# abhilash1910/bitsandbytes-SYCL

Measured on AMD Instinct MI355X. Metric: NF4 matmul TFLOPS + INT8 igemmlt TOPS @ 4096x4096x11008, 1/2/4/8 GPU, higher is better.
Workload: dtype bf16; 1 GPU; NF4 Linear4bit GEMM M=4096 N=4096 K=11008 (functional.gemm_4bit on its static route for 4096 x 4096 x 11008: k_hgemm<bf16> (hand-written, hgemm.hip) after k_dequantize_4bit_stream<bf16,NF4>, every step dequantising its weight); M=4096, N=4096, K=11008, blocksize=64, quant_type=nf4, compress_statistics=True, parallelism=single GPU

## Files before the change

bitsandbytes-sycl_amd/csrc/common.hpp:

```cpp
#pragma once

#include <hip/hip_runtime.h>
#include <atomic>
#include <stdint.h>
#include <stdio.h>

typedef uint16_t bf16_t;
typedef _Float16 fp16_t;

namespace bnb {

template <typename T> using Knob = std::atomic<T>;

enum DataType { GENERAL8BIT = 0, FP4 = 1, NF4 = 2 };

hipStream_t current_stream();
void set_error(int code, const char* what);
#define BNB_LAUNCH_CHECK(name)                                              \
  do {                                                                      \
    hipError_t e_ = hipGetLastError();                                      \
    if (e_ != hipSuccess) ::bnb::set_error((int)e_, name);                  \
  } while (0)

template <typename T> struct Io;
template <> struct Io<float> {
  __device__ static __forceinline__ float to_f32(float v) { return v; }
  __device__ static __forceinline__ float from_f32(float v) { return v; }
};
__device__ __forceinline__ float opaque(float v) {
  asm volatile("" : "+v"(v));
  return v;
// ... 225 lines not shown
```

bitsandbytes-sycl_amd/csrc/hgemm.hip:

```cpp
#include "gemm_common.hpp"
#include "int8_common.hpp"

#include <algorithm>
#include <type_traits>
#include <utility>

namespace bnb {

constexpr int HG_BM = 256, HG_BN = 256, HG_THREADS = 256;

typedef float hg_f32x2_t __attribute__((ext_vector_type(2)));
typedef __bf16 hg_bf16x2_t __attribute__((ext_vector_type(2)));
typedef _Float16 hg_f16x2_t __attribute__((ext_vector_type(2)));
template <typename T> __device__ __forceinline__ uint32_t cvt_pk(float lo, float hi);
template <> __device__ __forceinline__ uint32_t cvt_pk<bf16_t>(float lo, float hi) {
  return __builtin_bit_cast(uint32_t, __builtin_convertvector((hg_f32x2_t){lo, hi}, hg_bf16x2_t));
}
template <> __device__ __forceinline__ uint32_t cvt_pk<fp16_t>(float lo, float hi) {
  return __builtin_bit_cast(uint32_t, __builtin_convertvector((hg_f32x2_t){lo, hi}, hg_f16x2_t));
}

enum HgOp { HG_BF16 = 0, HG_FP16 = 1, HG_I8_DEQ = 2 };
typedef unsigned hg_u32x4_t __attribute__((ext_vector_type(4)));
typedef int hg_i32x4_t __attribute__((ext_vector_type(4)));
// ... 35 lines not shown
    acc_t c;
    asm volatile("v_mfma_i32_16x16x64_i8 %0, %1, %2, 0" : "=a"(c) : "v"(a), "v"(b));
    return c;
  }
};

__device__ __forceinline__ void glds16_sv_m0(const void* sbase, uint32_t voff, uint32_t lds) {
  asm volatile("s_mov_b32 m0, %2\n\ts_nop 0\n\tglobal_load_lds_dwordx4 %0, %1" : : "v"(voff), "s"(sbase), "s"(lds) : "memory");
}

template <int STEP>
__device__ __forceinline__ void glds16_chain(const void* sbase, uint32_t voff) {
  asm volatile("global_load_lds_dwordx4 %0, %1\n\ts_add_u32 m0, m0, %2" : : "v"(voff), "s"(sbase), "i"(STEP) : "memory");
}
__device__ __forceinline__ void hg_set_m0(uint32_t lds) { asm volatile("s_mov_b32 m0, %0" : : "s"(lds) : "memory"); }

__device__ __forceinline__ int hg_swz(int r, int s) { return r * 128 + ((s ^ ((r >> 1) & 7)) << 4); }

__device__ __forceinline__ void glds4_sv_m0(const void* sbase, uint32_t voff, uint32_t lds) {
  asm volatile("s_mov_b32 m0, %2\n\ts_nop 0\n\tglobal_load_lds_dword %0, %1" : : "v"(voff), "s"(sbase), "s"(lds) : "memory");
}

__device__ __forceinline__ uint32_t mm_dequant_pair(int32_t a0, int32_t a1, float rs, float cs0, float cs1, float b0,
                                                    float b1) {
  hg_f32x2_t v = {(float)a0, (float)a1};
  v = v * (hg_f32x2_t){6.200012e-05f, 6.200012e-05f};
  v = v * (hg_f32x2_t){rs, rs};
  v = v * (hg_f32x2_t){cs0, cs1};
  asm volatile("" : "+v"(v));
  v = v + (hg_f32x2_t){b0, b1};
// ... 4 lines not shown
constexpr int HG_V = 16 + 8192;
constexpr int HG_V_CWT = 32768;
static Knob<int> g_hg_cwt{1};
constexpr int HG_V_EPI = 65536;
static Knob<int> g_hg_epi{1};
constexpr int HG_V_CNT = 131072;
constexpr int HG_V_TL = 262144;
__device__ unsigned long long* g_hg_tl = nullptr;
__device__ int g_hg_tl_nswap = 0;
__device__ int g_hg_tl_nostore = 0;
[[maybe_unused]] static int g_hg_tl_on = 0;
__device__ __forceinline__ unsigned long long hg_now() {
  unsigned long long t;
  asm volatile("s_memrealtime %0\n\ts_waitcnt lgkmcnt(0)" : "=s"(t)::"memory");
  return t;
}

template <class F, int... Q>
__device__ __forceinline__ void hg_static_for_impl(F&& f, std::integer_sequence<int, Q...>) {
  (f(std::integral_constant<int, Q>{}), ...);
}
template <int N, class F>
__device__ __forceinline__ void hg_static_for(F&& f) {
  hg_static_for_impl(f, std::make_integer_sequence<int, N>{});
}

template <int WI, int WJ> struct HgPlan3;
template <> struct HgPlan3<8, 8> {
  static constexpr int B1 = 21, B2 = 50, B3 = 88, SETB = 22, SETA = 61, VM = 13, SIDEQ = 120;
  __host__ __device__ static constexpr int wread(int q) { return q < 16 && (q & 1) == 0 ? q >> 1 : -1; }
// ... 235 lines not shown
  const int first_m = (wg / group_span) * GROUP;
  const int gsize = min(tilesM - first_m, GROUP);
  const int tm = first_m + (wg % group_span) % gsize;
  int tn = (wg % group_span) / gsize;
  if constexpr (TL) {
    if (g_hg_tl_nswap) tn = (tn + tilesN / 2) % tilesN;
  }
  const int m0 = tm * BM, n0 = tn * BN;

  uint32_t aoff[WI], boff[WJ];
  const uint32_t lda2 = (uint32_t)lda * E, ldb2 = (uint32_t)ldb * E;
#pragma unroll
  for (int i = 0; i < WI; ++i) {
    const int row = 8 * (WI * wave + i) + (lane >> 3);
    const uint32_t slot = (uint32_t)((lane & 7) ^ ((row >> 1) & 7));
    aoff[i] = (uint32_t)min(m0 + row, M - 1) * lda2 + 16u * slot;
  }
#pragma unroll
  for (int i = 0; i < WJ; ++i) {
    const int row = 8 * (WJ * wave + i) + (lane >> 3);
    const uint32_t slot = (uint32_t)((lane & 7) ^ ((row >> 1) & 7));
    boff[i] = (uint32_t)min(n0 + row, N - 1) * ldb2 + 16u * slot;
  }
  const uint32_t lds_base = __builtin_amdgcn_readfirstlane((uint32_t)(uintptr_t)smem);
  const uint32_t ldsA0 = lds_base + wave * WI * 1024, ldsB0 = lds_base + TA + wave * WJ * 1024;
  auto dma_a = [&](int kt, int st, int i) { glds16_sv_m0(A + (long long)kt * 128, aoff[i], ldsA0 + st * STG + i * 1024); };
  auto dma_b = [&](int kt, int st, int i) { glds16_sv_m0(B + (long long)kt * 128, boff[i], ldsB0 + st * STG + i * 1024); };

  const int wm = wave >> 1, wn = wave & 1;
  const int fr = lane & 15, fg = lane >> 4, key = (fr >> 1) & 7;
  const int xo0 = (16 * WI * wm + fr) * 128 + ((fg ^ key) << 4);
  const int xo1 = (16 * WI * wm + fr) * 128 + (((4 + fg) ^ key) << 4);
  const int wo0 = TA + (16 * WJ * wn + fr) * 128 + ((fg ^ key) << 4);
  const int wo1 = TA + (16 * WJ * wn + fr) * 128 + (((4 + fg) ^ key) << 4);
  using frag_t = hg_u32x4_t;
  auto rd = [&](int st, int off, int f) -> frag_t {
    return *reinterpret_cast<const frag_t*>(smem + st * STG + off + f * 2048);
// ... 82 lines not shown
        glds4_sv_m0(bias, 4u * (uint32_t)min(n0 / 2 + 64 * c + lane, N / 2 - 1), sb + 4 * BM + 4 * BN + 256 * c);
  }
#pragma unroll
  for (int i = 0; i < WI; ++i) dma_a(0, 0, i);
#pragma unroll
  for (int i = 0; i < WJ; ++i) dma_b(0, 0, i);
  const int k1 = min(1, nk - 1);
#pragma unroll
  for (int i = 0; i < WI; ++i) dma_a(k1, 1, i);
#pragma unroll
  for (int i = 0; i < WJ; ++i) dma_b(k1, 1, i);
  asm volatile("s_waitcnt vmcnt(%0)" ::"i"(WI + WJ) : "memory");
  if constexpr (SIDE) __builtin_amdgcn_s_waitcnt(0xC07F);
  __builtin_amdgcn_s_barrier();
  if constexpr (TL) tl1 = hg_now();
#pragma unroll
  for (int f = 0; f < WJ; ++f) w0[f] = rd(0, wo0, f);
#pragma unroll
  for (int f = 0; f < WI; ++f) x0[f] = rd(0, xo0, f);

  if (nk == 1) {
    tile3(std::true_type{}, std::true_type{}, 0);
  } else {
    tile3(std::true_type{}, std::false_type{}, 0);
    for (int t = 1; t + 1 < nk; ++t) tile3(std::false_type{}, std::false_type{}, t);
    tile3(std::false_type{}, std::true_type{}, nk - 1);
  }
  wait_vmcnt0();
  if constexpr (TL) tl2 = hg_now();
  __builtin_amdgcn_sched_barrier(0);
  asm volatile("s_nop 7\n\ts_nop 7\n\ts_nop 7" ::: "memory");
  __builtin_amdgcn_sched_barrier(0);
  if constexpr (SIDE) {
    auto consume = [&](int it) {
      side_words(it);
      side_stat();
#pragma unroll
      for (int j = 0; j < 4; ++j) {
// ... 61 lines not shown
#pragma unroll
      for (int i = 0; i < WI; ++i) rsv[i] = *reinterpret_cast<const float*>(sst + 4 * (rl + 16 * i));
#pragma unroll
      for (int j = 0; j < WJ; ++j) {
        csv[j] = *reinterpret_cast<const f32x4_t*>(sst + 4 * BM + 4 * (cl + 16 * j));
        if ((N & 1) == 0)
          bsv[j] = bias ? *reinterpret_cast<const uint2*>(sst + 4 * BM + 4 * BN + 2 * (cl + 16 * j)) : make_uint2(0u, 0u);
        else
          bsv[j] = bias ? *reinterpret_cast<const uint2*>(bias + nb + 16 * j) : make_uint2(0u, 0u);
      }
    }
    auto convert = [&](int i, int j) {
      uint2 v;
      if constexpr (OP == HG_BF16 || OP == HG_FP16) {
        using T = typename std::conditional<OP == HG_BF16, bf16_t, fp16_t>::type;
        v.x = cvt_pk<T>(acc[j][i][0], acc[j][i][1]);
        v.y = cvt_pk<T>(acc[j][i][2], acc[j][i][3]);
      } else if constexpr (OP == HG_I8_DEQ) {
        auto bf = [&](uint32_t w, int hi) { return (float)__builtin_bit_cast(fp16_t, (uint16_t)(w >> (16 * hi))); };
        v.x = mm_dequant_pair(acc[j][i][0], acc[j][i][1], rsv[i], csv[j][0], csv[j][1], bf(bsv[j].x, 0), bf(bsv[j].x, 1));
        v.y = mm_dequant_pair(acc[j][i][2], acc[j][i][3], rsv[i], csv[j][2], csv[j][3], bf(bsv[j].y, 0), bf(bsv[j].y, 1));
      }
      *reinterpret_cast<uint2*>(ep + (16 * i + (lane_e & 15)) * EPI_PITCH + 2 * (16 * j + 4 * (lane_e >> 4))) = v;
    };
    uint8_t* cbase = reinterpret_cast<uint8_t*>(Cv) + ((long long)(m0 + 16 * WI * wm) * ldc + n0 + 16 * WJ * wn) * 2;
    constexpr int CPR = 2 * WJ, RPI = 64 / CPR;
    auto store_rows = [&](int it) {
      const int row = RPI * it + lane_e / CPR, c16 = lane_e % CPR;
      const uint4 v = *reinterpret_cast<const uint4*>(ep + row * EPI_PITCH + 16 * c16);
      uint8_t* dst = cbase + (long long)row * ldc * 2 + 16 * c16;
      if constexpr ((V & HG_V_CWT) != 0)
        asm volatile("global_store_dwordx4 %0, %1, off sc1" : : "v"(dst), "v"((hg_u32x4_t){v.x, v.y, v.z, v.w}) : "memory");
      else
        *reinterpret_cast<uint4*>(dst) = v;
    };
    if ((V & HG_V_EPI) != 0 && (long long)ldc * 2 * 16 * WI < 0x7FFFFFFFLL) {
// ... 42 lines not shown
          __builtin_amdgcn_sched_barrier(0);
        }
      }
      __builtin_amdgcn_s_waitcnt(0xC07F);
#pragma unroll 8
      for (int it = 0; it < 16 * WI / RPI; ++it) store_rows(it);
    }
  } else if (!full) {
#pragma unroll
    for (int i = 0; i < WI; ++i) {
      const int m = mb + 16 * i;
      const long long mc = min(m, M - 1);
      float rs = 0.f;
      if constexpr (OP == HG_I8_DEQ) rs = rowStats[mc];
#pragma unroll
      for (int j = 0; j < WJ; ++j)
#pragma unroll
        for (int r = 0; r < 4; ++r) {
          const int n = nb + 16 * j + r;
          if (m < M && n < N) {
            if constexpr (OP == HG_BF16) reinterpret_cast<bf16_t*>(Cv)[mc * ldc + n] = Io<bf16_t>::from_f32(acc[j][i][r]);
            else if constexpr (OP == HG_FP16) reinterpret_cast<fp16_t*>(Cv)[mc * ldc + n] = Io<fp16_t>::from_f32(acc[j][i][r]);
            else
              reinterpret_cast<fp16_t*>(Cv)[mc * ldc + n] =
                  mm_dequant_value(acc[j][i][r], rs, colStats[n], bias ? (float)bias[n] : 0.0f);
          }
          __builtin_amdgcn_sched_barrier(0);
        }
    }
  }
  if constexpr ((V & HG_V_TAIL) != 0) {
    __builtin_amdgcn_s_barrier();
    hg_side_tail<T16>(side, smem + wave * (16 * WI * EPI_PITCH), lane_e, blockIdx.x * 4u + (uint32_t)wave,
                      gridDim.x * 4u);
  }
  if constexpr (TL) {
    const unsigned long long tl3 = hg_now();
    asm volatile("s_waitcnt vmcnt(0)" ::: "memory");
    const unsigned long long tl4 = hg_now();
    if (lane == 0 && g_hg_tl != nullptr) {
      unsigned long long* o = g_hg_tl + ((long long)blockIdx.x * 4 + wave) * 8;
      o[0] = tl0; o[1] = tl1; o[2] = tl2; o[3] = tl3; o[4] = tl4; o[5] = (unsigned long long)wgs;
      o[6] = (unsigned long long)(__builtin_amdgcn_s_getreg((3 << 11) | 20) & 15);
// ... 289 lines not shown
```

bitsandbytes-sycl_amd/csrc/quant.hip:

```cpp
#include "common.hpp"

#include <type_traits>

namespace bnb {


template <typename T> struct Load8;
template <> struct Load8<float> {
  __device__ static __forceinline__ void load(const float* p, float (&v)[8]) {
    const float4 a = *reinterpret_cast<const float4*>(p);
    const float4 b = *reinterpret_cast<const float4*>(p + 4);
    v[0] = a.x; v[1] = a.y; v[2] = a.z; v[3] = a.w; v[4] = b.x; v[5] = b.y; v[6] = b.z; v[7] = b.w;
  }
};
template <> struct Load8<fp16_t> {
  __device__ static __forceinline__ void load(const fp16_t* p, float (&v)[8]) {
    const uint4 u = *reinterpret_cast<const uint4*>(p);
    const uint32_t w[4] = {u.x, u.y, u.z, u.w};
#pragma unroll
    for (int i = 0; i < 4; ++i) {
      v[2 * i] = (float)__builtin_bit_cast(fp16_t, (uint16_t)(w[i] & 0xFFFF));
      v[2 * i + 1] = (float)__builtin_bit_cast(fp16_t, (uint16_t)(w[i] >> 16));
    }
  }
// ... 412 lines not shown
}

template <typename T, int DT>
bool dequantize_4bit_nested(const uint8_t* A, const uint8_t* q8, const float* code2, const float* absmax2,
                            const float* offset, T* out, int blocksize, int blocksize2, long long n) {
  if (n <= 0) return true;
  if (blocksize < 64 || (blocksize & (blocksize - 1)) || blocksize2 <= 0 || (blocksize2 & (blocksize2 - 1)) ||
      n % 8 != 0 || ((uintptr_t)A & 3) != 0 || !aligned16(out))
    return false;
  const NestedStats ns{q8, code2, absmax2, offset, __builtin_ctz(blocksize2)};
  launch_dq_stream<T, DT, true>(A, nullptr, out, __builtin_ctz(blocksize), n / 8, ns);
  BNB_LAUNCH_CHECK("dequantize_4bit_nested");
  return true;
}

__global__ void __launch_bounds__(256)
k_dequantize_nested_absmax(const float* __restrict__ code2, const uint8_t* __restrict__ q, const float* __restrict__ absmax2,
                           const float* __restrict__ offset, float* __restrict__ out, int bs2_shift, long long n) {
  __shared__ float c2[256];
  c2[threadIdx.x] = code2[threadIdx.x];
  const float off = *offset;
  __syncthreads();
  const long long i0 = 16 * ((long long)blockIdx.x * 256 + threadIdx.x);
  if (i0 >= n) return;
  if (i0 + 16 <= n && (((uintptr_t)(q + i0)) & 15) == 0 && (((uintptr_t)(out + i0)) & 15) == 0) {
    const uint4 v = *reinterpret_cast<const uint4*>(q + i0);
    const uint32_t w[4] = {v.x, v.y, v.z, v.w};
#pragma unroll
    for (int d = 0; d < 4; ++d) {
      float r[4];
// ... 63 lines not shown
BNB_DEQUANT_ABI(cdequantize_blockwise_fp32_fp4, float, FP4)
BNB_DEQUANT_ABI(cdequantize_blockwise_fp32_nf4, float, NF4)

#define BNB_DEQUANT_NESTED_ABI(fname, T, DT)                                                                    \
  int fname(unsigned char* A, unsigned char* absmax_q, float* code2, float* absmax2, float* offset, T* out,      \
            int blocksize, int blocksize2, long long n) {                                                        \
    BNB_RANGE(#fname);                                                                                            \
    return dequantize_4bit_nested<T, DT>(A, absmax_q, code2, absmax2, offset, out, blocksize, blocksize2, n) ? 0  \
                                                                                                             : 1; \
  }
BNB_DEQUANT_NESTED_ABI(cdequantize_blockwise_nested_fp16_fp4, fp16_t, FP4)
BNB_DEQUANT_NESTED_ABI(cdequantize_blockwise_nested_fp16_nf4, fp16_t, NF4)
BNB_DEQUANT_NESTED_ABI(cdequantize_blockwise_nested_bf16_fp4, bf16_t, FP4)
BNB_DEQUANT_NESTED_ABI(cdequantize_blockwise_nested_bf16_nf4, bf16_t, NF4)


void cquantize_blockwise_bytes_fp32(float* code, float* A, float* absmax, unsigned char* out, long long blocksize,
                                    long long n) {
  BNB_RANGE("cquantize_blockwise_bytes_fp32");
  if (n <= 0 || blocksize <= 0) return;
  const long long nb = (n + blocksize - 1) / blocksize;
  if (nb > 0x7fffffffLL) { set_error(1, "quantize_bytes: too many blocks"); return; }
  hipLaunchKernelGGL(k_quantize_cpu_semantics, dim3((unsigned)nb), dim3(256), 0, current_stream(), code, A, absmax,
                     out, blocksize, n);
  BNB_LAUNCH_CHECK("quantize_bytes");
}

void cdequantize_nested_absmax_fp32(float* code2, unsigned char* q, float* absmax2, float* offset, float* out,
                                    int blocksize2, long long n) {
  BNB_RANGE("cdequantize_nested_absmax_fp32");
// ... 22 lines not shown
```

bitsandbytes-sycl_amd/csrc/runtime.hip:

```cpp
#include "common.hpp"

#include <atomic>
#include <cstdio>
#include <cstdlib>
#include <cstring>
#include <mutex>

#include <dlfcn.h>

namespace bnb {

static thread_local hipStream_t g_stream = nullptr;
static std::atomic<int> g_last_error{0};
static std::mutex g_err_mu;
static char g_err_msg[256] = {0};

hipStream_t current_stream() { return g_stream; }

void set_error(int code, const char* what) {
  g_last_error.store(code);
  std::lock_guard<std::mutex> lk(g_err_mu);
  std::snprintf(g_err_msg, sizeof(g_err_msg), "%s (code %d)", what, code);
  if (std::getenv("BNB_HIP_VERBOSE")) std::fprintf(stderr, "[bnb-hip] %s\n", g_err_msg);
}

typedef int (*roctx_push_fn)(const char*);
typedef int (*roctx_pop_fn)();
struct RoctxApi {
  roctx_push_fn push = nullptr;
  roctx_pop_fn pop = nullptr;
  RoctxApi() {
    const char* e = std::getenv("BNB_ROCTX");
// ... 46 lines not shown
  int concurrent = 0;
  hipDeviceGetAttribute(&concurrent, hipDeviceAttributeConcurrentManagedAccess, device);
  if (!concurrent) return;
  hipMemPrefetchAsync(ptr, bytes, device, bnb::current_stream());
}

void cset_stream(void* stream) { bnb::g_stream = (hipStream_t)stream; }
void* cget_stream() { return (void*)bnb::g_stream; }

int cget_last_error() { return bnb::g_last_error.exchange(0); }

const char* cget_last_error_message() { return bnb::g_err_msg; }

int cget_abi_version() { return 1; }

int croctx_enabled() { return bnb::roctx_api().push != nullptr ? 1 : 0; }

}
```

bitsandbytes-sycl_amd/python_src_quants/cextension.py:

```python
from __future__ import annotations

import ctypes as ct
import logging
import os
from pathlib import Path

logger = logging.getLogger(__name__)

PACKAGE_DIR = Path(__file__).parent
LIBRARY_NAME = "libbitsandbytes_hip.so"


def get_hip_bnb_library_path() -> Path:
    override = os.environ.get("BNB_HIP_LIBRARY")
    return Path(override) if override else PACKAGE_DIR / LIBRARY_NAME


class BNBNativeLibrary:
    _lib: ct.CDLL
    compiled_with_hip = True

    def __init__(self, lib: ct.CDLL):
        self._lib = lib
        lib.get_context.restype = ct.c_void_p
        lib.get_cusparse.restype = ct.c_void_p
        lib.cget_managed_ptr.restype = ct.c_void_p
        lib.cget_stream.restype = ct.c_void_p
        lib.cget_last_error_message.restype = ct.c_char_p
        lib.cgemm_4bit_workspace_bytes.restype = ct.c_longlong
        lib.cigemmlt_workspace_bytes.restype = ct.c_longlong
        lib.chgemm_tn_workspace_bytes.restype = ct.c_longlong
        lib.cipc_allgather_buffer_bytes.restype = ct.c_longlong
        lib.cipc_alloc.restype = ct.c_void_p
        lib.cipc_alloc.argtypes = [ct.c_longlong, ct.POINTER(ct.c_int)]
        for name in ("cigemmlt_turing_32", "cigemmlt_turing_8", "cigemmlt_turing_8_rowscale",
                     "cigemmlt_ampere_32", "cigemmlt_ampere_8", "cigemmlt_ampere_8_rowscale",
                     "cigemmlt_row_dequant_fp16", "cigemm_row_i32", "cigemmlt_row_dequant_ws_fp16",
                     "cigemm_row_i32_ws", "cgemm_tn_bf16", "cgemm_tn_fp16", "cgemm_tn_set_search", "cgemm_tn_plan",
                     "chgemm_tn_bf16", "chgemm_tn_fp16", "cprobe_mfma", "cprobe_hbm_read",
                     "cget_last_error", "cget_abi_version",
                     "cgemm_4bit_inference_naive_nested_fp16", "cgemm_4bit_inference_naive_nested_bf16",
                     "cdequantize_blockwise_nested_fp16_fp4", "cdequantize_blockwise_nested_fp16_nf4",
                     "cdequantize_blockwise_nested_bf16_fp4", "cdequantize_blockwise_nested_bf16_nf4",
                     "cint8_row_quant_fp16", "cgemm_4bit_inference_nested_ws_bf16",
                     "cgemm_4bit_inference_nested_ws_fp16", "cset_cpu_threads", "cgemm_4bit_fewtok_takes", "chgemm_tn_ws_bf16", "chgemm_tn_ws_fp16",
                     "cipc_handle_size", "cipc_get_handle", "cipc_open_handle", "cipc_close_handle", "callgather_ipc_16",
                     "cprobe_lds_poison", "cprobe_lds_peek", "croctx_enabled"):
# ... 38 lines not shown
```

bitsandbytes-sycl_amd/python_src_quants/functional.py:

```python
from __future__ import annotations

import ctypes as ct
import functools
import os
import threading
import weakref
from functools import reduce
import operator
from typing import Any, Dict, Optional, Tuple

import torch
from torch import Tensor

from .cextension import lib
from .utils import pack_dict_to_tensor, unpack_tensor_to_dict

name2qmap: Dict[str, Tensor] = {}

dtype2bytes = {torch.float32: 4, torch.float16: 2, torch.bfloat16: 2, torch.uint8: 1, torch.int8: 1}

_BLOCKSIZES = [4096, 2048, 1024, 512, 256, 128, 64]


def prod(iterable):
# ... 854 lines not shown
    return bool(lib.cgemm_4bit_fewtok_takes(ct.c_int32(n), ct.c_int32(rows), ct.c_int32(k), ct.c_int32(blocksize)))


_FEWTOK_MODE = [0]


def set_fewtok_mode(mode: int) -> None:
    lib.cgemm_4bit_set_fewtok_mode(ct.c_int(mode))
    _FEWTOK_MODE[0] = mode


_EVENT_POOL: list = []


def reserve_stage_events(n: int) -> None:
    for _ in range(n):
        e = torch.cuda.Event(enable_timing=True)
        e.record()
        _EVENT_POOL.append(e)
    torch.cuda.synchronize()


def _stage_events(n: int) -> list:
    return [_EVENT_POOL.pop() if _EVENT_POOL else torch.cuda.Event(enable_timing=True) for _ in range(n)]


def _gemm_4bit_tokens(A2: Tensor, Bc: Tensor, state: QuantState, out: Tensor, absmax: Optional[Tensor],
                      events: Optional[list]) -> bool:
    N, K = state.shape[0], state.shape[1]
    rows = A2.shape[0]
    nested = absmax is None and _nested_stats_in_kernel_ok(state)
# ... 58 lines not shown
        s2 = sn.state2
        stats = [None, sn.absmax, s2.code, s2.absmax, _offset_on(sn, A2.device)]
        bs2 = s2.blocksize
    else:
        stats = [an if an is not None else _absmax_fp32(sn), None, None, None, None]
        bs2 = 0
    Bc = Bn
    is_on_gpu([Bc, target] + [t for t in stats if t is not None])
    fn = lib.chgemm_tn_pf_bf16 if A2.dtype == torch.bfloat16 else lib.chgemm_tn_pf_fp16
    return fn(ct.c_int32(rows), ct.c_int32(N), ct.c_int32(K), get_ptr(A2), ct.c_int32(K), get_ptr(W), ct.c_int32(K),
              get_ptr(out), ct.c_int32(N), get_ptr(ws), ct.c_longlong(ws_bytes), get_ptr(Bc),
              *[get_ptr(t) for t in stats], ct.c_int32(1 if sn.quant_type == "fp4" else 0), ct.c_int32(sn.blocksize),
              ct.c_int32(bs2), ct.c_longlong(sn.shape[0] * sn.shape[1]), get_ptr(target))


def gemm_4bit(A: Tensor, B: Tensor, state: QuantState, out: Optional[Tensor] = None,
              absmax: Optional[Tensor] = None, events: Optional[list] = None, reuse_weight: bool = False,
              _route: Optional[str] = None, prefetch: Optional[tuple] = None) -> Tensor:
    if not gemm_4bit_supported(A, state):
        raise ValueError("gemm_4bit: needs bf16/fp16 activations and in_features % 64 == 0")
    N, K = state.shape[0], state.shape[1]
    A2 = A.reshape(-1, K)
    if not A2.is_contiguous() or A2.data_ptr() % 16:
        A2 = A2.contiguous()
    rows = A2.shape[0]
    if out is None:
        out = torch.empty((rows, N), dtype=A.dtype, device=A.device)
    Bc = B if B.is_contiguous() else B.contiguous()
    if prefetch is not None and not prefetch[0].is_contiguous():
        prefetch = None
    route = gemm_4bit_static_route(rows, N, K)
    if _route is not None:
        if _route not in GEMM_4BIT_ROUTES:
            raise ValueError(f"gemm_4bit: unknown route {_route!r}")
        route = _route
    elif GEMM_4BIT_ROUTE_TUNING and rows > GEMM_4BIT_FEW_TOKENS:
# ... 44 lines not shown
    is_on_gpu([A2, Bc, out, state.code] + ([absmax] if absmax is not None else []))
    ev = _stage_events(3) if events is not None else None
    if ev:
        ev[0].record()
    if library:
        key = (A.device, A.dtype, _stream_key(A.device))
        meta = _weight_meta(Bc, state, absmax)
        ready = _PF_READY.get(key)
        cur_slot = None
        if ready is not None and ready[1] == meta:
            cur_slot = ready[0]
            del _PF_READY[key]
            _PF_CUR[key] = ready
        elif reuse_weight and _PF_CUR.get(key, (None, None))[1] == meta:
            cur_slot = _PF_CUR[key][0]
        if cur_slot is not None:
            W = _PF_WS[key][cur_slot][:N * K].view(N, K)
        else:
            W = _dequant_workspace(A.device, A.dtype, N * K).view(N, K)
        if cur_slot is None and not (reuse_weight and _DEQ_META.get(key) == meta):
            if absmax is None and not _dequant_4bit_nested(Bc, state, W):
                absmax = _absmax_fp32(state)
            if absmax is not None:
                qt = "fp4" if state.quant_type == "fp4" else "nf4"
                getattr(lib, f"cdequantize_blockwise_{_QB[A.dtype]}_{qt}")(
                    get_ptr(None), get_ptr(Bc), get_ptr(absmax), get_ptr(W), ct.c_int(state.blocksize),
                    ct.c_int(N * K))
            _DEQ_META[key] = meta
            if ev:
                ev[1].record()
                events.append(("dequantize", ev[0], ev[1]))
        elif ev:
            ev[1].record()
        if route == "hgemm":
            ws_bytes = int(lib.chgemm_tn_workspace_bytes(ct.c_int32(rows), ct.c_int32(N), ct.c_int32(K)))
            ws = _gemm_workspace(A.device, ws_bytes)
            rc = 1
            if prefetch is not None:
                sn = prefetch[1]
                nn = sn.shape[0] * sn.shape[1]
                slots = _pf_slots(key, A.device, A.dtype, max(nn, N * K))
                target = 1 - cur_slot if cur_slot is not None else 0
                rc = _launch_prefetch_gemm(A2, W, out, ws, ws_bytes, prefetch, slots[target][:nn])
                if rc == 0:
                    if _PF_CUR.get(key, (None,))[0] == target:
                        _PF_CUR.pop(key, None)
                    _PF_READY[key] = (target, _weight_meta(prefetch[0], sn, prefetch[2] if len(prefetch) > 2 else None))
            if rc == 1:
                fn = lib.chgemm_tn_ws_bf16 if A.dtype == torch.bfloat16 else lib.chgemm_tn_ws_fp16
                rc = fn(ct.c_int32(rows), ct.c_int32(N), ct.c_int32(K), get_ptr(A2), ct.c_int32(K), get_ptr(W),
                        ct.c_int32(K), get_ptr(out), ct.c_int32(N), get_ptr(ws), ct.c_longlong(ws_bytes))
            post_call(prev_device)
            if rc:
                raise RuntimeError(f"bitsandbytes HIP GEMM (chgemm_tn) returned {rc}: "
                                   f"{lib.cget_last_error_message().decode() if rc == 2 else 'shape not supported'}")
        elif route == "library_tn":
            fn = lib.cgemm_tn_bf16 if A.dtype == torch.bfloat16 else lib.cgemm_tn_fp16
            rc = fn(ct.c_int32(rows), ct.c_int32(N), ct.c_int32(K), get_ptr(A2), ct.c_int32(K), get_ptr(W),
                    ct.c_int32(K), get_ptr(out), ct.c_int32(N))
            post_call(prev_device)
            if rc:
                raise RuntimeError(f"bitsandbytes HIP library GEMM error: {lib.cget_last_error_message().decode()}")
        else:
            post_call(prev_device)
            torch.matmul(A2, W.t(), out=out.view(rows, N))
        if ev:
            ev[2].record()
            events.append(("gemm", ev[1], ev[2]))
        return out.view(*A.shape[:-1], N)
    ws_bytes = int(lib.cgemm_4bit_workspace_bytes(ct.c_int32(N), ct.c_int32(rows), ct.c_int32(K)))
    ws = _gemm_workspace(A.device, ws_bytes)
    fn = lib.cgemm_4bit_inference_code_ws_bf16 if A.dtype == torch.bfloat16 else lib.cgemm_4bit_inference_code_ws_fp16
    fn(ct.c_int32(N), ct.c_int32(rows), ct.c_int32(K), get_ptr(A2), get_ptr(Bc), get_ptr(absmax),
       get_ptr(state.code), get_ptr(out), ct.c_int32(K), ct.c_int32((K + 1) // 2), ct.c_int32(N),
       ct.c_int32(state.blocksize), get_ptr(ws), ct.c_longlong(ws_bytes))
    post_call(prev_device)
    if ev:
        ev[2].record()
        events.append(("gemm", ev[0], ev[2]))
    return out.view(*A.shape[:-1], N)


def get_transform_buffer(shape, dtype, device, to_order, from_order="row", transpose=False):
# ... 392 lines not shown
```

include/bnb_hip.h:

```cpp
#ifndef BNB_HIP_H
#define BNB_HIP_H

#include <stddef.h>
#include <stdint.h>
#include <stdbool.h>

#ifdef __cplusplus
extern "C" {
#endif

typedef unsigned short bnb_fp16;
typedef unsigned short bnb_bf16;

void* get_context(void);
void* get_cusparse(void);
void* cget_managed_ptr(size_t bytes);
void cprefetch(void* ptr, size_t bytes, int device);

void cquantize_blockwise_fp16(float* code, bnb_fp16* A, float* absmax, unsigned char* out, int blocksize, const int n);
void cquantize_blockwise_fp16_fp4(float* code, bnb_fp16* A, float* absmax, unsigned char* out, int blocksize, const int n);
void cquantize_blockwise_fp16_nf4(float* code, bnb_fp16* A, float* absmax, unsigned char* out, int blocksize, const int n);
void cquantize_blockwise_fp32(float* code, float* A, float* absmax, unsigned char* out, int blocksize, const int n);
void cquantize_blockwise_fp32_fp4(float* code, float* A, float* absmax, unsigned char* out, int blocksize, const int n);
void cquantize_blockwise_fp32_nf4(float* code, float* A, float* absmax, unsigned char* out, int blocksize, const int n);
// ... 201 lines not shown
        float weight_decay, const float gnorm_scale, bool skip_zeros, int n);
void clion_8bit_blockwise_grad_fp16(bnb_fp16* p, bnb_fp16* g, unsigned char* state1, unsigned char* state2, float beta1, float beta2,
        float eps, int step, float lr, float* quantiles1, float* quantiles2, float* absmax1, float* absmax2,
        float weight_decay, const float gnorm_scale, bool skip_zeros, int n);
void clion_8bit_blockwise_grad_bf16(bnb_bf16* p, bnb_bf16* g, unsigned char* state1, unsigned char* state2, float beta1, float beta2,
        float eps, int step, float lr, float* quantiles1, float* quantiles2, float* absmax1, float* absmax2,
        float weight_decay, const float gnorm_scale, bool skip_zeros, int n);
int cdequantize_blockwise_nested_fp16_fp4(unsigned char* A, unsigned char* absmax_q, float* code2, float* absmax2,
        float* offset, bnb_fp16* out, int blocksize, int blocksize2, long long n);
int cdequantize_blockwise_nested_fp16_nf4(unsigned char* A, unsigned char* absmax_q, float* code2, float* absmax2,
        float* offset, bnb_fp16* out, int blocksize, int blocksize2, long long n);
int cdequantize_blockwise_nested_bf16_fp4(unsigned char* A, unsigned char* absmax_q, float* code2, float* absmax2,
        float* offset, bnb_bf16* out, int blocksize, int blocksize2, long long n);
int cdequantize_blockwise_nested_bf16_nf4(unsigned char* A, unsigned char* absmax_q, float* code2, float* absmax2,
        float* offset, bnb_bf16* out, int blocksize, int blocksize2, long long n);
void cadam32bit_grad_fp32(float* g, float* p, float* state1, float* state2, float* unorm, float max_unorm,
        float param_norm, const float beta1, const float beta2, const float eps, const float weight_decay,
        const int step, const float lr, const float gnorm_scale, bool skip_zeros, const int n);
void cadam32bit_grad_fp16(bnb_fp16* g, bnb_fp16* p, float* state1, float* state2, float* unorm, float max_unorm,
        float param_norm, const float beta1, const float beta2, const float eps, const float weight_decay,
        const int step, const float lr, const float gnorm_scale, bool skip_zeros, const int n);
void cadam32bit_grad_bf16(bnb_bf16* g, bnb_bf16* p, float* state1, float* state2, float* unorm, float max_unorm,
        float param_norm, const float beta1, const float beta2, const float eps, const float weight_decay,
        const int step, const float lr, const float gnorm_scale, bool skip_zeros, const int n);
void cmomentum32bit_grad_32(float* g, float* p, float* state1, float* state2, float* unorm, float max_unorm,
        float param_norm, const float beta1, const float beta2, const float eps, const float weight_decay,
        const int step, const float lr, const float gnorm_scale, bool skip_zeros, const int n);
void cmomentum32bit_grad_16(bnb_fp16* g, bnb_fp16* p, float* state1, float* state2, float* unorm, float max_unorm,
        float param_norm, const float beta1, const float beta2, const float eps, const float weight_decay,
        const int step, const float lr, const float gnorm_scale, bool skip_zeros, const int n);
// ... 60 lines not shown
```

Before: 1508 TFLOP/s.

## Add opt-in dequantise-ahead side stream and tweak hgemm accumulator reads

Adds an opt-in path that dequantises the NF4 weight on a low-priority side stream into double-buffered slots, using events to order it against the main stream so the dequant can overlap the previous GEMM. Alongside this, the hgemm kernel now reads accumulators with explicit v_accvgpr_read instructions in the epilogue, hides row-offset multiplies from the compiler, and refactors the first fragment load. The side-stream path only runs when BNB_DEQUANT_AHEAD=1, so by default only the kernel codegen tweaks apply. The overlap path adds event and stream bookkeeping plus risk around slot reuse.

```diff
diff --git a/bitsandbytes-sycl_amd/csrc/common.hpp b/bitsandbytes-sycl_amd/csrc/common.hpp
--- a/bitsandbytes-sycl_amd/csrc/common.hpp
+++ b/bitsandbytes-sycl_amd/csrc/common.hpp
@@ -15,6 +15,15 @@
 enum DataType { GENERAL8BIT = 0, FP4 = 1, NF4 = 2 };
 
 hipStream_t current_stream();
+struct StreamScope {
+  hipStream_t prev;
+  explicit StreamScope(hipStream_t s);
+  ~StreamScope();
+  StreamScope(const StreamScope&) = delete;
+  StreamScope& operator=(const StreamScope&) = delete;
+};
+hipStream_t ahead_begin(int slot, bool behind_main);
+int ahead_ready(int slot);
 void set_error(int code, const char* what);
 #define BNB_LAUNCH_CHECK(name)                                              \
   do {                                                                      \
diff --git a/bitsandbytes-sycl_amd/csrc/hgemm.hip b/bitsandbytes-sycl_amd/csrc/hgemm.hip
--- a/bitsandbytes-sycl_amd/csrc/hgemm.hip
+++ b/bitsandbytes-sycl_amd/csrc/hgemm.hip
@@ -73,6 +73,12 @@
   asm volatile("global_load_lds_dwordx4 %0, %1\n\ts_add_u32 m0, m0, %2" : : "v"(voff), "s"(sbase), "i"(STEP) : "memory");
 }
 __device__ __forceinline__ void hg_set_m0(uint32_t lds) { asm volatile("s_mov_b32 m0, %0" : : "s"(lds) : "memory"); }
+
+__device__ __forceinline__ uint32_t hg_row_off(uint32_t row, uint32_t ld, uint32_t add) {
+  uint32_t p = row * ld;
+  asm volatile("" : "+v"(p));
+  return p + add;
+}
 
 __device__ __forceinline__ int hg_swz(int r, int s) { return r * 128 + ((s ^ ((r >> 1) & 7)) << 4); }
 
@@ -107,6 +113,12 @@
   unsigned long long t;
   asm volatile("s_memrealtime %0\n\ts_waitcnt lgkmcnt(0)" : "=s"(t)::"memory");
   return t;
+}
+
+template <typename A, typename S>
+__device__ __forceinline__ void hg_acc_read(const A& a, S (&f)[4]) {
+#pragma unroll
+  for (int r = 0; r < 4; ++r) asm volatile("v_accvgpr_read_b32 %0, %1" : "=v"(f[r]) : "a"(a[r]));
 }
 
 template <class F, int... Q>
@@ -372,13 +384,13 @@
   for (int i = 0; i < WI; ++i) {
     const int row = 8 * (WI * wave + i) + (lane >> 3);
     const uint32_t slot = (uint32_t)((lane & 7) ^ ((row >> 1) & 7));
-    aoff[i] = (uint32_t)min(m0 + row, M - 1) * lda2 + 16u * slot;
+    aoff[i] = hg_row_off((uint32_t)min(m0 + row, M - 1), lda2, 16u * slot);
   }
 #pragma unroll
   for (int i = 0; i < WJ; ++i) {
     const int row = 8 * (WJ * wave + i) + (lane >> 3);
     const uint32_t slot = (uint32_t)((lane & 7) ^ ((row >> 1) & 7));
-    boff[i] = (uint32_t)min(n0 + row, N - 1) * ldb2 + 16u * slot;
+    boff[i] = hg_row_off((uint32_t)min(n0 + row, N - 1), ldb2, 16u * slot);
   }
   const uint32_t lds_base = __builtin_amdgcn_readfirstlane((uint32_t)(uintptr_t)smem);
   const uint32_t ldsA0 = lds_base + wave * WI * 1024, ldsB0 = lds_base + TA + wave * WJ * 1024;
@@ -491,14 +503,20 @@
   if constexpr (SIDE) __builtin_amdgcn_s_waitcnt(0xC07F);
   __builtin_amdgcn_s_barrier();
   if constexpr (TL) tl1 = hg_now();
-#pragma unroll
-  for (int f = 0; f < WJ; ++f) w0[f] = rd(0, wo0, f);
-#pragma unroll
-  for (int f = 0; f < WI; ++f) x0[f] = rd(0, xo0, f);
+  auto frag0 = [&](int z) {
+#pragma unroll
+    for (int f = 0; f < WJ; ++f) w0[f] = rd(0, wo0 + z, f);
+#pragma unroll
+    for (int f = 0; f < WI; ++f) x0[f] = rd(0, xo0 + z, f);
+  };
 
   if (nk == 1) {
+    int z = 0;
+    asm volatile("" : "+v"(z));
+    frag0(z);
     tile3(std::true_type{}, std::true_type{}, 0);
   } else {
+    frag0(0);
     tile3(std::true_type{}, std::false_type{}, 0);
     for (int t = 1; t + 1 < nk; ++t) tile3(std::false_type{}, std::false_type{}, t);
     tile3(std::false_type{}, std::true_type{}, nk - 1);
@@ -590,12 +608,16 @@
       uint2 v;
       if constexpr (OP == HG_BF16 || OP == HG_FP16) {
         using T = typename std::conditional<OP == HG_BF16, bf16_t, fp16_t>::type;
-        v.x = cvt_pk<T>(acc[j][i][0], acc[j][i][1]);
-        v.y = cvt_pk<T>(acc[j][i][2], acc[j][i][3]);
+        float f[4];
+        hg_acc_read(acc[j][i], f);
+        v.x = cvt_pk<T>(f[0], f[1]);
+        v.y = cvt_pk<T>(f[2], f[3]);
       } else if constexpr (OP == HG_I8_DEQ) {
         auto bf = [&](uint32_t w, int hi) { return (float)__builtin_bit_cast(fp16_t, (uint16_t)(w >> (16 * hi))); };
-        v.x = mm_dequant_pair(acc[j][i][0], acc[j][i][1], rsv[i], csv[j][0], csv[j][1], bf(bsv[j].x, 0), bf(bsv[j].x, 1));
-        v.y = mm_dequant_pair(acc[j][i][2], acc[j][i][3], rsv[i], csv[j][2], csv[j][3], bf(bsv[j].y, 0), bf(bsv[j].y, 1));
+        int32_t a[4];
+        hg_acc_read(acc[j][i], a);
+        v.x = mm_dequant_pair(a[0], a[1], rsv[i], csv[j][0], csv[j][1], bf(bsv[j].x, 0), bf(bsv[j].x, 1));
+        v.y = mm_dequant_pair(a[2], a[3], rsv[i], csv[j][2], csv[j][3], bf(bsv[j].y, 0), bf(bsv[j].y, 1));
       }
       *reinterpret_cast<uint2*>(ep + (16 * i + (lane_e & 15)) * EPI_PITCH + 2 * (16 * j + 4 * (lane_e >> 4))) = v;
     };
@@ -668,19 +690,22 @@
       float rs = 0.f;
       if constexpr (OP == HG_I8_DEQ) rs = rowStats[mc];
 #pragma unroll
-      for (int j = 0; j < WJ; ++j)
+      for (int j = 0; j < WJ; ++j) {
+        typename std::conditional<OP == HG_I8_DEQ, int32_t, float>::type f[4];
+        hg_acc_read(acc[j][i], f);
 #pragma unroll
         for (int r = 0; r < 4; ++r) {
           const int n = nb + 16 * j + r;
           if (m < M && n < N) {
-            if constexpr (OP == HG_BF16) reinterpret_cast<bf16_t*>(Cv)[mc * ldc + n] = Io<bf16_t>::from_f32(acc[j][i][r]);
-            else if constexpr (OP == HG_FP16) reinterpret_cast<fp16_t*>(Cv)[mc * ldc + n] = Io<fp16_t>::from_f32(acc[j][i][r]);
+            if constexpr (OP == HG_BF16) reinterpret_cast<bf16_t*>(Cv)[mc * ldc + n] = Io<bf16_t>::from_f32(f[r]);
+            else if constexpr (OP == HG_FP16) reinterpret_cast<fp16_t*>(Cv)[mc * ldc + n] = Io<fp16_t>::from_f32(f[r]);
             else
               reinterpret_cast<fp16_t*>(Cv)[mc * ldc + n] =
-                  mm_dequant_value(acc[j][i][r], rs, colStats[n], bias ? (float)bias[n] : 0.0f);
+                  mm_dequant_value(f[r], rs, colStats[n], bias ? (float)bias[n] : 0.0f);
           }
           __builtin_amdgcn_sched_barrier(0);
         }
+      }
     }
   }
   if constexpr ((V & HG_V_TAIL) != 0) {
diff --git a/bitsandbytes-sycl_amd/csrc/quant.hip b/bitsandbytes-sycl_amd/csrc/quant.hip
--- a/bitsandbytes-sycl_amd/csrc/quant.hip
+++ b/bitsandbytes-sycl_amd/csrc/quant.hip
@@ -450,6 +450,32 @@
   return true;
 }
 
+template <typename T, int DT>
+int dequantize_4bit_ahead(const uint8_t* A, const float* absmax, const uint8_t* q8, const float* code2,
+                          const float* absmax2, const float* offset, T* out, int blocksize, int blocksize2, long long n,
+                          int slot, bool behind_main) {
+  const bool nested = q8 != nullptr;
+  if (n <= 0 || blocksize < 64 || (blocksize & (blocksize - 1)) || n % 8 != 0 || ((uintptr_t)A & 3) != 0 || !aligned16(out))
+    return 1;
+  if (nested ? (!code2 || !absmax2 || !offset || blocksize2 <= 0 || (blocksize2 & (blocksize2 - 1))) : !absmax) return 1;
+  const hipStream_t side = ahead_begin(slot, behind_main);
+  if (side == nullptr) return 1;
+  {
+    StreamScope on_side(side);
+    if (nested)
+      launch_dq_stream<T, DT, true>(A, nullptr, out, __builtin_ctz(blocksize), n / 8,
+                                    NestedStats{q8, code2, absmax2, offset, __builtin_ctz(blocksize2)});
+    else
+      launch_dq_stream<T, DT, false>(A, absmax, out, __builtin_ctz(blocksize), n / 8, NestedStats{});
+  }
+  const hipError_t e = hipGetLastError();
+  if (e != hipSuccess) {
+    set_error((int)e, "dequantize_4bit_ahead");
+    return 2;
+  }
+  return ahead_ready(slot) ? 2 : 0;
+}
+
 __global__ void __launch_bounds__(256)
 k_dequantize_nested_absmax(const float* __restrict__ code2, const uint8_t* __restrict__ q, const float* __restrict__ absmax2,
                            const float* __restrict__ offset, float* __restrict__ out, int bs2_shift, long long n) {
@@ -543,6 +569,18 @@
 BNB_DEQUANT_NESTED_ABI(cdequantize_blockwise_nested_bf16_fp4, bf16_t, FP4)
 BNB_DEQUANT_NESTED_ABI(cdequantize_blockwise_nested_bf16_nf4, bf16_t, NF4)
 
+#define BNB_DEQUANT_AHEAD_ABI(fname, T, DT)                                                                        \
+  int fname(unsigned char* A, float* absmax, unsigned char* absmax_q, float* code2, float* absmax2, float* offset,  \
+            T* out, int blocksize, int blocksize2, long long n, int slot, int behind_main) {                        \
+    BNB_RANGE(#fname);                                                                                               \
+    return dequantize_4bit_ahead<T, DT>(A, absmax, absmax_q, code2, absmax2, offset, out, blocksize, blocksize2, n,  \
+                                        slot, behind_main != 0);                                                     \
+  }
+BNB_DEQUANT_AHEAD_ABI(cdequantize_4bit_ahead_fp16_fp4, fp16_t, FP4)
+BNB_DEQUANT_AHEAD_ABI(cdequantize_4bit_ahead_fp16_nf4, fp16_t, NF4)
+BNB_DEQUANT_AHEAD_ABI(cdequantize_4bit_ahead_bf16_fp4, bf16_t, FP4)
+BNB_DEQUANT_AHEAD_ABI(cdequantize_4bit_ahead_bf16_nf4, bf16_t, NF4)
+
 
 void cquantize_blockwise_bytes_fp32(float* code, float* A, float* absmax, unsigned char* out, long long blocksize,
                                     long long n) {
diff --git a/bitsandbytes-sycl_amd/csrc/runtime.hip b/bitsandbytes-sycl_amd/csrc/runtime.hip
--- a/bitsandbytes-sycl_amd/csrc/runtime.hip
+++ b/bitsandbytes-sycl_amd/csrc/runtime.hip
@@ -4,7 +4,9 @@
 #include <cstdio>
 #include <cstdlib>
 #include <cstring>
+#include <map>
 #include <mutex>
+#include <utility>
 
 #include <dlfcn.h>
 
@@ -16,6 +18,78 @@
 static char g_err_msg[256] = {0};
 
 hipStream_t current_stream() { return g_stream; }
+
+StreamScope::StreamScope(hipStream_t s) : prev(g_stream) { g_stream = s; }
+StreamScope::~StreamScope() { g_stream = prev; }
+
+struct AheadLane {
+  hipStream_t side = nullptr;
+  hipEvent_t fork = nullptr;
+  hipEvent_t free_ev[2] = {nullptr, nullptr}, ready_ev[2] = {nullptr, nullptr};
+  bool free_set[2] = {false, false}, ready_set[2] = {false, false};
+};
+static std::mutex g_ahead_mu;
+static std::map<std::pair<int, hipStream_t>, AheadLane*> g_ahead;
+
+static AheadLane* ahead_lane(bool create) {
+  int dev = 0;
+  if (hipGetDevice(&dev) != hipSuccess) return nullptr;
+  std::lock_guard<std::mutex> lk(g_ahead_mu);
+  auto it = g_ahead.find({dev, g_stream});
+  if (it != g_ahead.end()) return it->second;
+  if (!create) return nullptr;
+  auto* l = new AheadLane();
+  int lo = 0, hi = 0;
+  hipDeviceGetStreamPriorityRange(&lo, &hi);
+  bool ok = hipStreamCreateWithPriority(&l->side, hipStreamNonBlocking, lo) == hipSuccess;
+  ok = ok && hipEventCreateWithFlags(&l->fork, hipEventDisableTiming) == hipSuccess;
+  for (int s = 0; s < 2 && ok; ++s)
+    ok = hipEventCreateWithFlags(&l->free_ev[s], hipEventDisableTiming) == hipSuccess &&
+         hipEventCreateWithFlags(&l->ready_ev[s], hipEventDisableTiming) == hipSuccess;
+  if (!ok) {
+    (void)hipGetLastError();
+    set_error(2, "dequantise-ahead lane: stream / event creation failed");
+    delete l;
+    return nullptr;
+  }
+  g_ahead[{dev, g_stream}] = l;
+  return l;
+}
+
+static bool main_stream_capturing() {
+  hipStreamCaptureStatus st = hipStreamCaptureStatusNone;
+  if (hipStreamIsCapturing(g_stream, &st) != hipSuccess) {
+    (void)hipGetLastError();
+    return true;
+  }
+  return st != hipStreamCaptureStatusNone;
+}
+
+hipStream_t ahead_begin(int slot, bool behind_main) {
+  if (slot < 0 || slot > 1 || main_stream_capturing()) return nullptr;
+  AheadLane* l = ahead_lane(true);
+  if (!l) return nullptr;
+  bool ok = true;
+  if (behind_main)
+    ok = hipEventRecord(l->fork, g_stream) == hipSuccess && hipStreamWaitEvent(l->side, l->fork, 0) == hipSuccess;
+  if (ok && l->free_set[slot]) ok = hipStreamWaitEvent(l->side, l->free_ev[slot], 0) == hipSuccess;
+  if (!ok) {
+    set_error((int)hipGetLastError(), "dequantise-ahead: ordering the side stream");
+    return nullptr;
+  }
+  return l->side;
+}
+
+int ahead_ready(int slot) {
+  AheadLane* l = (slot < 0 || slot > 1) ? nullptr : ahead_lane(false);
+  if (!l) return 1;
+  if (hipEventRecord(l->ready_ev[slot], l->side) != hipSuccess) {
+    set_error((int)hipGetLastError(), "dequantise-ahead: recording ready");
+    return 2;
+  }
+  l->ready_set[slot] = true;
+  return 0;
+}
 
 void set_error(int code, const char* what) {
   g_last_error.store(code);
@@ -92,6 +166,26 @@
 
 int cget_abi_version() { return 1; }
 
+void* cdequantize_4bit_ahead_begin(int slot, int behind_main) { return (void*)bnb::ahead_begin(slot, behind_main != 0); }
+int cdequantize_4bit_ahead_wait(int slot) {
+  bnb::AheadLane* l = (slot < 0 || slot > 1 || bnb::main_stream_capturing()) ? nullptr : bnb::ahead_lane(false);
+  if (!l || !l->ready_set[slot]) return 1;
+  if (hipStreamWaitEvent(bnb::g_stream, l->ready_ev[slot], 0) != hipSuccess) {
+    bnb::set_error((int)hipGetLastError(), "dequantise-ahead: waiting for ready");
+    return 2;
+  }
+  return 0;
+}
+int cdequantize_4bit_ahead_release(int slot) {
+  bnb::AheadLane* l = (slot < 0 || slot > 1 || bnb::main_stream_capturing()) ? nullptr : bnb::ahead_lane(true);
+  if (!l) return 1;
+  if (hipEventRecord(l->free_ev[slot], bnb::g_stream) != hipSuccess) {
+    bnb::set_error((int)hipGetLastError(), "dequantise-ahead: recording free");
+    return 2;
+  }
+  l->free_set[slot] = true;
+  return 0;
+}
 int croctx_enabled() { return bnb::roctx_api().push != nullptr ? 1 : 0; }
 
 }
diff --git a/bitsandbytes-sycl_amd/python_src_quants/cextension.py b/bitsandbytes-sycl_amd/python_src_quants/cextension.py
--- a/bitsandbytes-sycl_amd/python_src_quants/cextension.py
+++ b/bitsandbytes-sycl_amd/python_src_quants/cextension.py
@@ -31,6 +31,7 @@
         lib.cigemmlt_workspace_bytes.restype = ct.c_longlong
         lib.chgemm_tn_workspace_bytes.restype = ct.c_longlong
         lib.cipc_allgather_buffer_bytes.restype = ct.c_longlong
+        lib.cdequantize_4bit_ahead_begin.restype = ct.c_void_p
         lib.cipc_alloc.restype = ct.c_void_p
         lib.cipc_alloc.argtypes = [ct.c_longlong, ct.POINTER(ct.c_int)]
         for name in ("cigemmlt_turing_32", "cigemmlt_turing_8", "cigemmlt_turing_8_rowscale",
diff --git a/bitsandbytes-sycl_amd/python_src_quants/functional.py b/bitsandbytes-sycl_amd/python_src_quants/functional.py
--- a/bitsandbytes-sycl_amd/python_src_quants/functional.py
+++ b/bitsandbytes-sycl_amd/python_src_quants/functional.py
@@ -892,7 +892,7 @@
 
 
 def reserve_stage_events(n: int) -> None:
-    for _ in range(n):
+    for _ in range(n + (n + 2) // 3 if _AHEAD[0] else n):
         e = torch.cuda.Event(enable_timing=True)
         e.record()
         _EVENT_POOL.append(e)
@@ -981,12 +981,75 @@
               ct.c_int32(bs2), ct.c_longlong(sn.shape[0] * sn.shape[1]), get_ptr(target))
 
 
+_AHEAD = [os.environ.get("BNB_DEQUANT_AHEAD", "0") == "1"]
+_AHEAD_EPOCH = [0]
+
+
+def set_dequant_ahead(on: bool) -> bool:
+    prev = _AHEAD[0]
+    _AHEAD[0] = bool(on)
+    _AHEAD_EPOCH[0] += 1
+    return prev
+
+
+def _dequant_ahead(key, A: Tensor, Bc: Tensor, b_temp: bool, state: QuantState, absmax: Optional[Tensor],
+                   absmax_given: bool, meta: tuple, ev: Optional[list]) -> Optional[int]:
+    if torch.cuda.is_current_stream_capturing():
+        return None
+    device, dtype = A.device, A.dtype
+    N, K = state.shape[0], state.shape[1]
+    if absmax is None:
+        if not _nested_stats_in_kernel_ok(state):
+            return None
+        s2 = state.state2
+        offset = _offset_on(state, device)
+        stats = [None, state.absmax, s2.code, s2.absmax, offset]
+        bs2 = s2.blocksize
+        stable = offset is state.offset
+    else:
+        stats = [absmax, None, None, None, None]
+        bs2 = 0
+        stable = not absmax_given and absmax is state.absmax
+    ident = (key, _AHEAD_EPOCH[0], Bc.data_ptr(), Bc._version) + tuple(
+        x for t in stats if t is not None for x in (t.data_ptr(), t._version))
+    had = _PF_WS.get(key)
+    slots = _pf_slots(key, device, dtype, N * K)
+    cur = _PF_CUR.get(key)
+    slot = 1 - cur[0] if cur is not None else 0
+    behind = (b_temp or not stable or slots is not had or getattr(state, "_ahead_seen", None) != ident)
+    target = slots[slot][:N * K]
+    is_on_gpu([Bc, target] + [t for t in stats if t is not None])
+    side = None
+    if ev:
+        sp = lib.cdequantize_4bit_ahead_begin(ct.c_int32(slot), ct.c_int32(1 if behind else 0))
+        if not sp:
+            return None
+        side = torch.cuda.ExternalStream(sp, device=device)
+        ev[0].record(side)
+    qt = "fp4" if state.quant_type == "fp4" else "nf4"
+    rc = getattr(lib, f"cdequantize_4bit_ahead_{_QB[dtype]}_{qt}")(
+        get_ptr(Bc), *[get_ptr(t) for t in stats], get_ptr(target), ct.c_int32(state.blocksize), ct.c_int32(bs2),
+        ct.c_longlong(N * K), ct.c_int32(slot), ct.c_int32(1 if behind else 0))
+    if rc == 1:
+        return None
+    if rc == 0 and side is not None:
+        ev[1].record(side)
+    if rc or lib.cdequantize_4bit_ahead_wait(ct.c_int32(slot)):
+        raise RuntimeError(f"bitsandbytes HIP dequantise-ahead error: {lib.cget_last_error_message().decode()}")
+    state._ahead_seen = ident
+    _PF_CUR[key] = (slot, meta)
+    if _PF_READY.get(key, (None,))[0] == slot:
+        del _PF_READY[key]
+    return slot
+
+
 def gemm_4bit(A: Tensor, B: Tensor, state: QuantState, out: Optional[Tensor] = None,
               absmax: Optional[Tensor] = None, events: Optional[list] = None, reuse_weight: bool = False,
               _route: Optional[str] = None, prefetch: Optional[tuple] = None) -> Tensor:
     if not gemm_4bit_supported(A, state):
         raise ValueError("gemm_4bit: needs bf16/fp16 activations and in_features % 64 == 0")
     N, K = state.shape[0], state.shape[1]
+    absmax_given = absmax is not None
     A2 = A.reshape(-1, K)
     if not A2.is_contiguous() or A2.data_ptr() % 16:
         A2 = A2.contiguous()
@@ -1061,6 +1124,16 @@
             _PF_CUR[key] = ready
         elif reuse_weight and _PF_CUR.get(key, (None, None))[1] == meta:
             cur_slot = _PF_CUR[key][0]
+        ev_gemm = ev[1] if ev else None
+        if (cur_slot is None and route == "hgemm" and prefetch is None and _AHEAD[0]
+                and not (reuse_weight and _DEQ_META.get(key) == meta)):
+            cur_slot = _dequant_ahead(key, A, Bc, Bc is not B, state, absmax, absmax_given, meta, ev)
+            if cur_slot is not None and ev:
+                events.append(("dequantize", ev[0], ev[1]))
+                ev_gemm = _stage_events(1)[0]
+                ev_gemm.record()
+            elif ev:
+                ev[0].record()
         if cur_slot is not None:
             W = _PF_WS[key][cur_slot][:N * K].view(N, K)
         else:
@@ -1077,12 +1150,13 @@
             if ev:
                 ev[1].record()
                 events.append(("dequantize", ev[0], ev[1]))
-        elif ev:
+        elif ev and ev_gemm is ev[1]:
             ev[1].record()
         if route == "hgemm":
             ws_bytes = int(lib.chgemm_tn_workspace_bytes(ct.c_int32(rows), ct.c_int32(N), ct.c_int32(K)))
             ws = _gemm_workspace(A.device, ws_bytes)
             rc = 1
+            target = None
             if prefetch is not None:
                 sn = prefetch[1]
                 nn = sn.shape[0] * sn.shape[1]
@@ -1097,6 +1171,10 @@
                 fn = lib.chgemm_tn_ws_bf16 if A.dtype == torch.bfloat16 else lib.chgemm_tn_ws_fp16
                 rc = fn(ct.c_int32(rows), ct.c_int32(N), ct.c_int32(K), get_ptr(A2), ct.c_int32(K), get_ptr(W),
                         ct.c_int32(K), get_ptr(out), ct.c_int32(N), get_ptr(ws), ct.c_longlong(ws_bytes))
+            if _AHEAD[0] and rc == 0:
+                for s_ in (cur_slot, target):
+                    if s_ is not None:
+                        lib.cdequantize_4bit_ahead_release(ct.c_int32(s_))
             post_call(prev_device)
             if rc:
                 raise RuntimeError(f"bitsandbytes HIP GEMM (chgemm_tn) returned {rc}: "
@@ -1111,9 +1189,11 @@
         else:
             post_call(prev_device)
             torch.matmul(A2, W.t(), out=out.view(rows, N))
+        if route != "hgemm" and cur_slot is not None:
+            _AHEAD_EPOCH[0] += 1
         if ev:
             ev[2].record()
-            events.append(("gemm", ev[1], ev[2]))
+            events.append(("gemm", ev_gemm, ev[2]))
         return out.view(*A.shape[:-1], N)
     ws_bytes = int(lib.cgemm_4bit_workspace_bytes(ct.c_int32(N), ct.c_int32(rows), ct.c_int32(K)))
     ws = _gemm_workspace(A.device, ws_bytes)
diff --git a/include/bnb_hip.h b/include/bnb_hip.h
--- a/include/bnb_hip.h
+++ b/include/bnb_hip.h
@@ -239,6 +239,17 @@
         float* offset, bnb_bf16* out, int blocksize, int blocksize2, long long n);
 int cdequantize_blockwise_nested_bf16_nf4(unsigned char* A, unsigned char* absmax_q, float* code2, float* absmax2,
         float* offset, bnb_bf16* out, int blocksize, int blocksize2, long long n);
+int cdequantize_4bit_ahead_fp16_fp4(unsigned char* A, float* absmax, unsigned char* absmax_q, float* code2, float* absmax2,
+        float* offset, bnb_fp16* out, int blocksize, int blocksize2, long long n, int slot, int behind_main);
+int cdequantize_4bit_ahead_fp16_nf4(unsigned char* A, float* absmax, unsigned char* absmax_q, float* code2, float* absmax2,
+        float* offset, bnb_fp16* out, int blocksize, int blocksize2, long long n, int slot, int behind_main);
+int cdequantize_4bit_ahead_bf16_fp4(unsigned char* A, float* absmax, unsigned char* absmax_q, float* code2, float* absmax2,
+        float* offset, bnb_bf16* out, int blocksize, int blocksize2, long long n, int slot, int behind_main);
+int cdequantize_4bit_ahead_bf16_nf4(unsigned char* A, float* absmax, unsigned char* absmax_q, float* code2, float* absmax2,
+        float* offset, bnb_bf16* out, int blocksize, int blocksize2, long long n, int slot, int behind_main);
+int cdequantize_4bit_ahead_wait(int slot);
+int cdequantize_4bit_ahead_release(int slot);
+void* cdequantize_4bit_ahead_begin(int slot, int behind_main);
 void cadam32bit_grad_fp32(float* g, float* p, float* state1, float* state2, float* unorm, float max_unorm,
         float param_norm, const float beta1, const float beta2, const float eps, const float weight_decay,
         const int step, const float lr, const float gnorm_scale, bool skip_zeros, const int n);
```

Result: no change. 1510 TFLOP/s, median of 6 (+0.1%).
